# indygreg/python-zstandard

Hardware: NVIDIA H100
Metric: uncompressed GB/s (compress+decompress) (higher is better)
Workload: dtype u8

## Files before the change

### python_zstandard_b200/csrc/zb_common.cuh

```cuda
#pragma once
#include <cstdint>
#include <cstring>
#include <cuda_runtime.h>

typedef uint8_t  u8;
typedef uint16_t u16;
typedef uint32_t u32;
typedef uint64_t u64;

enum : u32 {
    ZB_OK = 0,
    ZB_E_GENERIC = 1,
    ZB_E_PREFIX_UNKNOWN = 10,
    ZB_E_FRAMEPARAM_UNSUPPORTED = 14,
    ZB_E_WINDOW_TOO_LARGE = 16,
    ZB_E_CORRUPTION = 20,
    ZB_E_CHECKSUM_WRONG = 22,
    ZB_E_LITERALS_HEADER_WRONG = 24,
    ZB_E_DICT_CORRUPTED = 30,
    ZB_E_DICT_WRONG = 32,
    ZB_E_TABLELOG_TOO_LARGE = 44,
    ZB_E_MAXSYMBOL_TOO_SMALL = 48,
    ZB_E_MEMORY = 64,
    ZB_E_DSTSIZE_TOO_SMALL = 70,
    ZB_E_SRCSIZE_WRONG = 72,
    ZB_E_UNKNOWN_SIZE = 200,
    ZB_E_SIZE_MISMATCH = 201,
};

#define ZB_MAGIC       0xFD2FB528u
#define ZB_MAGIC_DICT  0xEC30A437u
#define ZB_MAGIC_SKIP  0x184D2A50u
#define ZB_BLOCK_MAX   (128u << 10)
#define ZB_CONTENT_UNKNOWN 0xFFFFFFFFFFFFFFFFull

struct ZbSegment { u64 offset, length; };

#ifdef ZB_SIMT_EMULATION
#define ZB_LAUNCH(kernel, grid, block, smem, stream, ...) simt::launch((grid), (block), [&] { kernel(__VA_ARGS__); })
#else
#define ZB_LAUNCH(kernel, grid, block, smem, stream, ...) do { \
        if (smem) cudaFuncSetAttribute(kernel, cudaFuncAttributeMaxDynamicSharedMemorySize, (int)(smem)); \
        kernel<<<(grid), (block), (smem), (stream)>>>(__VA_ARGS__); } while (0)
#endif

static inline u32 zb_block_max(u32 window_log) { return window_log && window_log < 17 ? (1u << window_log) : ZB_BLOCK_MAX; }

template <class Seg, class JobVec, class InfoVec>
static inline u32 zb_cut_blocks(const Seg* segs, size_t n, u32 block_max, JobVec& jobs, InfoVec& info)
{
    u32 max_block = 0;
    for (size_t i = 0; i < n; i++) {
        u64 const len = segs[i].length; u64 pos = 0;
        info[i].first_job = jobs.size(); info[i].n_jobs = 0; info[i].pad = 0;
        while (pos < len) {
            u32 const sz = (u32)(len - pos < block_max ? len - pos : block_max);
            typename JobVec::value_type j;
            j.src_pos = segs[i].offset + pos; j.size = sz; j.seg = (u32)i; j.first = pos == 0; j.last = pos + sz == len;
            jobs.push_back(j); info[i].n_jobs++; pos += sz;
            if (sz > max_block) max_block = sz;
        }
    }
    return max_block;
}

static inline u64 zb_slot_bytes(u32 max_block) { return ((u64)max_block + (max_block >> 7) + 64 + 15) & ~15ull; }

struct ZbDictView { const u8* tail; u32 D; };
static inline ZbDictView zb_dict_view(const u8* content, u32 content_size)
{
    u32 const D = content_size < 32768u ? content_size : 32768u;
    ZbDictView v; v.tail = content + (content_size - D); v.D = D >= 8 ? D : 0;
    return v;
}

#define ZE_CHAIN_STEP 4u
static inline u64 zb_chain_positions(u64 len) { return len >= 8 ? (len - 8) / ZE_CHAIN_STEP + 1 : 0; }
static inline u32 zb_chain_log(u64 len)
{
    u64 const npos = zb_chain_positions(len);
    u32 L = 4; while ((1ull << L) < 4 * npos) L++;
    return L;
}
template <class Seg, class Desc, class JobVec, class InfoVec>
static inline void zb_chain_plan(const Seg* chunks, size_t m, Desc* cs, u64* tab_off, u64* pos_off, JobVec& jobs, InfoVec& info)
{
// ... 27 lines not shown
    return k > n_frames ? n_frames : k;
}
static inline u32 zb_chunk_cut(u32 n_frames, u32 k, u32 n_chunks) { return (u32)((u64)n_frames * k / n_chunks); }

struct ZbChunkShape { u32 warps, take, ctas; };
static inline ZbChunkShape zb_chunk_shape(u64 out_bytes, u32 n_frames, u32 sm_count)
{
    u64 const avg_out = out_bytes / (n_frames ? n_frames : 1);
    ZbChunkShape s;
    s.warps = avg_out <= (8u << 10) ? 8u : 7u;
    s.take = avg_out <= (8u << 10) ? 32u : (avg_out <= (16u << 10) ? 16u : (avg_out <= (32u << 10) ? 8u : (avg_out <= (64u << 10) ? 4u : 3u)));
    { u32 const spread = (n_frames + sm_count * s.warps - 1) / (sm_count * s.warps); if (s.take > spread) s.take = spread ? spread : 1; }
    s.ctas = sm_count; { u32 const need = (n_frames + s.warps * s.take - 1) / (s.warps * s.take); if (s.ctas > need) s.ctas = need; if (s.ctas == 0) s.ctas = 1; }
    return s;
}

struct ZbFrameInfo {
    u64 content_size;
    u64 n_seq_rec;
    u64 n_lit;
    u32 n_blocks;
    u32 status;
    u32 dict_id;
    u32 flags;
};

#define ZB_FAR_WINDOW  ((1ull << 31) - (1ull << 27))
#define ZB_FAR_DICT    (1ull << 27)

struct ZbFramePlace {
    u64 dst_off;
    u64 dst_cap;
    u64 blk_off;
    u64 seq_off;
    u64 lit_off;
};

enum : u32 { ZB_BLK_RAW = 0, ZB_BLK_RLE = 1, ZB_BLK_COMPRESSED = 2 };
enum : u32 { ZB_LIT_RAW = 0, ZB_LIT_RLE = 1, ZB_LIT_SCRATCH = 2 };

struct ZbBlock {
    u64 out_pos;
    u64 src_pos;
    u64 seq_pos;
    u32 kind;
    u32 regen;
    u32 lit_kind;
    u32 n_lit;
    u32 n_seq;
    u32 lit_byte;
};

typedef uint4 ZbSeq;

typedef u32 ZbFseCell;
#define ZB_CELL(next, nb, add, sym) ((u32)(next) | ((u32)(nb) << 10) | ((u32)(add) << 14) | ((u32)(sym) << 19))
#define ZB_CELL_NEXT(c) ((c) & 1023u)
#define ZB_CELL_NB(c)   (((c) >> 10) & 15u)
#define ZB_CELL_ADD(c)  (((c) >> 14) & 31u)
#define ZB_CELL_SYM(c)  ((c) >> 19)
#define ZB_CELL16(sym, x) ((u16)((sym) | ((x) << 6)))

struct ZbDictDev {
    const u8* content; u32 content_size; u32 dict_id;
    const u16* huf; u32 huf_log; u32 has_entropy;
    const ZbFseCell* ll; const ZbFseCell* of; const ZbFseCell* ml;
    u32 ll_log, of_log, ml_log;
    u32 rep[3];
};

struct ZbDictDigest {
    u16 huf[4096]; ZbFseCell ll[512]; ZbFseCell ml[512]; ZbFseCell of[256];
    u32 huf_log, ll_log, of_log, ml_log; u32 rep[3]; u32 dict_id; u32 content_off; u32 status; u32 has_entropy; u32 pad;
    short c_norm_ll[36], c_norm_of[32], c_norm_ml[54]; u32 c_max_ll, c_max_of, c_max_ml;
    u8 c_huf_nb[256]; u32 c_huf_max;
};

__device__ __forceinline__ u32 zb_rd16(const u8* p) { return (u32)p[0] | ((u32)p[1] << 8); }
__device__ __forceinline__ u32 zb_rd24(const u8* p) { return zb_rd16(p) | ((u32)p[2] << 16); }
__device__ __forceinline__ u32 zb_rd32(const u8* p) { return zb_rd16(p) | (zb_rd16(p + 2) << 16); }
__device__ __forceinline__ u64 zb_rd64(const u8* p) { return (u64)zb_rd32(p) | ((u64)zb_rd32(p + 4) << 32); }
__device__ __forceinline__ int zb_hibit(u32 v) { return 31 - __clz(v); }

__device__ __forceinline__ void zb_cp16(u8* sdst, const u8* gsrc)
{
#ifdef __CUDA_ARCH__
    asm volatile("cp.async.cg.shared.global [%0], [%1], 16;" :: "r"((u32)__cvta_generic_to_shared(sdst)), "l"(gsrc) : "memory");
#else
    memcpy(sdst, gsrc, 16);
#endif
}
__device__ __forceinline__ void zb_cp_commit()
{
#ifdef __CUDA_ARCH__
    asm volatile("cp.async.commit_group;" ::: "memory");
#endif
}
template <int N> __device__ __forceinline__ void zb_cp_wait()
{
#ifdef __CUDA_ARCH__
    asm volatile("cp.async.wait_group %0;" :: "n"(N) : "memory");
#endif
}

#ifdef __CUDA_ARCH__
#define ZB_RING_ARG(name) u8* name
#else
#define ZB_RING_ARG(name) u8* name = nullptr
#endif
template <int D>
struct ZbBitR {
    static_assert(D >= 2 && (D & (D - 1)) == 0, "ring depth: a power of two");
    const u8* c; u8* ring; int widx; u32 hi, lo; int avail; u32 nx0, nx1; int skew_bits; int lo_c; u32 n_;
#ifndef __CUDA_ARCH__
    alignas(16) u8 own[16 * D];
#endif

    __device__ __forceinline__ u32 word(int j) const { return *(const u32*)(ring + ((u32)j & (4u * D - 1)) * 4u); }
    __device__ __forceinline__ void fetch(int k) { zb_cp16(ring + ((u32)k & (D - 1)) * 16u, c + 16 * k); }
    __device__ __forceinline__ ~ZbBitR() { zb_cp_wait<0>(); }

    __device__ __forceinline__ bool start(const u8* s, u32 n, u8* ring_) {
        if (n == 0) return false;
#ifdef __CUDA_ARCH__
        ring = ring_;
#else
        ring = ring_ ? ring_ : own;
#endif
        c = (const u8*)((uintptr_t)s & ~(uintptr_t)15);
        int const skew = (int)(s - c);
        skew_bits = skew * 8; n_ = n;
        int const top = (skew + (int)n - 1) >> 4;
        #pragma unroll
        for (int q = 0; q < D; q++) if (top - q >= 0) fetch(top - q);
        zb_cp_commit();
        lo_c = top - D + 1 > 0 ? top - D + 1 : 0;
        return true;
    }
    __device__ __forceinline__ bool finish() {
        zb_cp_wait<0>();
        int const e = skew_bits / 8 + (int)n_ - 1;
        u32 const last = ring[(u32)e & (16u * D - 1)];
        if (last == 0) return false;
        int const P = e * 8 + zb_hibit(last);
        nx0 = nx1 = 0; lo = 0;
        if (P == 0) { hi = 0; avail = 0; widx = -1; return true; }
        int const wi = (P - 1) >> 5, k = P - wi * 32;
        hi = word(wi) << (32 - k); avail = k; widx = wi - 1;
        if (widx >= 0) nx0 = word(widx);
        if (widx >= 1) nx1 = word(widx - 1);
        refill();
        return true;
    }
    __device__ __forceinline__ bool init(const u8* s, u32 n, u8* ring_) { return start(s, n, ring_) && finish(); }
    __device__ __forceinline__ void refill() {
        zb_cp_wait<4 * D - 8>();
        bool const r = (avail <= 32) & (widx >= 0);
        u32 const a = (u32)avail;
        u32 const add_hi = __funnelshift_rc(nx0, 0u, a);
        u32 const new_lo = __funnelshift_lc(0u, nx0, 32u - a);
        hi |= r ? add_hi : 0u;
        lo = r ? new_lo : lo;
        avail += r ? 32 : 0;
        widx -= r ? 1 : 0;
        nx0 = r ? nx1 : nx0;
        if (r && widx >= 1) nx1 = word(widx - 1);
        int const t = ((widx - 1) >> 2) + 1 - D;
        if (t >= 0 && t < lo_c) { fetch(t); lo_c = t; }
        zb_cp_commit();
    }
    __device__ __forceinline__ u32 peek(u32 nb) const { return __funnelshift_rc(hi, 0u, 32u - nb); }
    __device__ __forceinline__ void skip(u32 nb) {
        hi = __funnelshift_lc(lo, hi, nb); lo = __funnelshift_lc(0u, lo, nb); avail -= (int)nb;
    }
    __device__ __forceinline__ u32 read(u32 nb) { u32 const v = peek(nb); skip(nb); return v; }
    __device__ __forceinline__ int left() const { return avail + 32 * (widx + 1) - skew_bits; }
};
```

### python_zstandard_b200/csrc/zb_entropy.cuh

```cuda
#pragma once

#define ZB_ENT_WS_BYTES   256
#define ZB_ENT_WS_STRIDE  (ZB_ENT_WS_BYTES + 16)
#define ZB_ENT_SKEW(b)    ((((b) + 15u) & ~15u) | 16u)
#define ZB_ENT_DEF_LL     512
#define ZB_ENT_DEF_OF     (ZB_ENT_DEF_LL + 2 * 64)
#define ZB_ENT_DEF_ML     (ZB_ENT_DEF_OF + 2 * 32)
#define ZB_ENT_HEAD_BYTES (ZB_ENT_DEF_ML + 2 * 64)
#define ZB_ENT_POOL_BYTES(W) ((((227 * 1024 - ZB_ENT_HEAD_BYTES) / (W))) & ~15)
#define ZB_ENT_SMEM(W)    ((W) * ZB_ENT_POOL_BYTES(W) + ZB_ENT_HEAD_BYTES)

enum : u32 { ZB_SRC_NONE = 0, ZB_SRC_PREDEF = 1, ZB_SRC_RLE = 2, ZB_SRC_NCOUNT = 3, ZB_SRC_DICT = 4 };
struct ZbTabSrc { u32 kind; u32 sym; const u8* p; u32 n; };

enum : u32 { ZB_BD_FIRST = 1, ZB_BD_FSE_VALID = 2, ZB_BD_SKIP = 4 };
struct ZbBlkDesc {
    u64 hdr_off;
    u64 seq_off, lit_off;
    u32 span;
    u32 frame;
    u32 flags;
    u32 block_max;
    ZbTabSrc dHuf, dLL, dOF, dML;
};
// ... 94 lines not shown
#define ZB_HUF_COARSE 8u
struct ZbHufTab { const u16* cells; u32 log, shift, T, base; };
__device__ __forceinline__ void zb_huf_shape(u32 log, ZbRank const& rank, u32& shift, u32& T, u32& base, u32& bytes)
{
    shift = log > ZB_HUF_COARSE ? log - ZB_HUF_COARSE : 0u;
    T = 0;
    #pragma unroll
    for (u32 wt = 1; wt <= 12 - ZB_HUF_COARSE; wt++) T += wt <= shift ? rank[wt] << (wt - 1) : 0u;
    base = (T + 3u) & ~3u;
    bytes = 2u * (base + (1u << (log - shift)));
}
__device__ __forceinline__ ZbHufTab zb_huf_full(const u16* cells, u32 log) { ZbHufTab t; t.cells = cells; t.log = log; t.shift = 0; t.T = 0; t.base = 0; return t; }
#define ZB_HCELL(t, v) ((t).cells[(v) < (t).T ? (v) : (t).base + ((v) >> (t).shift)])

__device__ static void zb_huf_fill(u16* cells, const u8* ws, u32 log, u32 nsym, ZbRank const& rank, u32 shift, u32 base)
{
    ZbPacked<6, 16> next; next.clear();
    {
        u32 p = 0;
        #pragma unroll
        for (u32 wt = 1; wt <= 12; wt++) { next.add(wt - 1, p); p += wt <= log ? (rank[wt] << (wt - 1)) : 0; }
    }
    for (u32 i = 0; i < nsym; i++) {
        u32 const wt = (ws[i >> 1] >> ((i & 1) * 4)) & 15; if (!wt) continue;
        u32 len = 1u << (wt - 1), p = next.get(wt - 1); next.add(wt - 1, len);
        if (wt > shift) { len >>= shift; p = base + (p >> shift); }
        u32 const cell = i | ((log + 1 - wt) << 8);
        if (len >= 4) { u64 const v = cell * 0x0001000100010001ull; u64* q = (u64*)(cells + p); for (u32 k = 0; k < len / 4; k++) q[k] = v; }
        else if (len == 2) *(u32*)(cells + p) = cell * 0x00010001u;
        else cells[p] = (u16)cell;
    }
}

#ifdef ZB_SIMT_EMULATION
__device__ __forceinline__ ZbRank zb_rank_pack(const u32* rank) { ZbRank r; r.clear(); for (u32 wt = 1; wt <= 12; wt++) r.add(wt - 1, rank[wt]); return r; }
__device__ static u32 zb_huf_weights(u8* ws, const u8* s, u32 n, u32& out_log, u32& out_nsym, u32* rank, ZB_RING_ARG(ring))
{
    ZbRank r; u32 const used = zb_huf_weights(ws, s, n, out_log, out_nsym, r, ring);
    rank[0] = used ? out_nsym : 0;
    for (u32 w = 1; w <= 12; w++) { rank[w] = used ? r[w] : 0; rank[0] -= rank[w]; }
    return used;
}
__device__ __forceinline__ void zb_huf_shape(u32 log, const u32* rank, u32& shift, u32& T, u32& base, u32& bytes)
{
    zb_huf_shape(log, zb_rank_pack(rank), shift, T, base, bytes);
}
__device__ static void zb_huf_fill(u16* cells, const u8* ws, u32 log, u32 nsym, const u32* rank, u32 shift, u32 base)
{
    zb_huf_fill(cells, ws, log, nsym, zb_rank_pack(rank), shift, base);
}
#endif

__device__ static bool zb_huf_stream2(u8* out, u32 n_out, const u8* s, u32 n, ZbHufTab const t, u8* ring)
{
    ZbBitR<4> b;
    if (!b.init(s, n, ring)) return false;
    u32 const log = t.log;
    u32 i = 0;
    while (i < n_out && ((uintptr_t)(out + i) & 3)) { u32 v = b.peek(log); u32 c = ZB_HCELL(t, v); out[i++] = (u8)c; b.skip(c >> 8); b.refill(); }
    for (; i + 4 <= n_out; i += 4) {
        u32 v0 = b.peek(log); u32 c0 = ZB_HCELL(t, v0); b.skip(c0 >> 8);
        u32 v1 = b.peek(log); u32 c1 = ZB_HCELL(t, v1); b.skip(c1 >> 8); b.refill();
        u32 v2 = b.peek(log); u32 c2 = ZB_HCELL(t, v2); b.skip(c2 >> 8);
        u32 v3 = b.peek(log); u32 c3 = ZB_HCELL(t, v3); b.skip(c3 >> 8); b.refill();
        *(u32*)(out + i) = (c0 & 255) | ((c1 & 255) << 8) | ((c2 & 255) << 16) | (c3 << 24);
    }
    for (; i < n_out; i++) { u32 v = b.peek(log); u32 c = ZB_HCELL(t, v); out[i] = (u8)c; b.skip(c >> 8); b.refill(); }
    return b.left() == 0;
}

struct ZbHufLane { ZbBitR<4> b; u8* out; u32 left; };

__device__ __forceinline__ void zb_huf_one(ZbHufLane& h, ZbHufTab const& t)
{
    u32 const v = h.b.peek(t.log); u32 const c = ZB_HCELL(t, v); *h.out++ = (u8)c; h.b.skip(c >> 8); h.b.refill(); h.left--;
}
#define ZB_HUF4(h) do { \
        u32 const v0_ = h.b.peek(t.log); u32 const c0_ = ZB_HCELL(t, v0_); h.b.skip(c0_ >> 8); \
        u32 const v1_ = h.b.peek(t.log); u32 const c1_ = ZB_HCELL(t, v1_); h.b.skip(c1_ >> 8); h.b.refill(); \
        u32 const v2_ = h.b.peek(t.log); u32 const c2_ = ZB_HCELL(t, v2_); h.b.skip(c2_ >> 8); \
        u32 const v3_ = h.b.peek(t.log); u32 const c3_ = ZB_HCELL(t, v3_); h.b.skip(c3_ >> 8); h.b.refill(); \
        *(u32*)h.out = (c0_ & 255) | ((c1_ & 255) << 8) | ((c2_ & 255) << 16) | (c3_ << 24); h.out += 4; h.left -= 4; } while (0)

__device__ static bool zb_huf_block(u8* dstl, u32 regen, const u8* p, u32 left, bool single, ZbHufTab const t, ZB_RING_ARG(ring))
{
    if (single) return zb_huf_stream2(dstl, regen, p, left, t, ring);
    if (left < 10) return false;
    u32 const l1 = zb_rd16(p), l2 = zb_rd16(p + 2), l3 = zb_rd16(p + 4), seg = (regen + 3) / 4;
    if (6 + l1 + l2 + l3 > left || seg * 3 > regen) return false;
    u32 const l4 = left - 6 - l1 - l2 - l3;
    ZbHufLane h0, h1, h2, h3;
    u8* const r1 = ring ? ring + 64 : nullptr; u8* const r2 = ring ? ring + 128 : nullptr; u8* const r3 = ring ? ring + 192 : nullptr;
    if (!h0.b.start(p + 6, l1, ring) || !h1.b.start(p + 6 + l1, l2, r1) || !h2.b.start(p + 6 + l1 + l2, l3, r2) || !h3.b.start(p + 6 + l1 + l2 + l3, l4, r3)) return false;
    if (!h0.b.finish() || !h1.b.finish() || !h2.b.finish() || !h3.b.finish()) return false;
    h0.out = dstl; h1.out = dstl + seg; h2.out = dstl + 2 * seg; h3.out = dstl + 3 * seg;
    h0.left = h1.left = h2.left = seg; h3.left = regen - 3 * seg;
    while (h0.left && ((uintptr_t)h0.out & 3)) zb_huf_one(h0, t);
    while (h1.left && ((uintptr_t)h1.out & 3)) zb_huf_one(h1, t);
    while (h2.left && ((uintptr_t)h2.out & 3)) zb_huf_one(h2, t);
    while (h3.left && ((uintptr_t)h3.out & 3)) zb_huf_one(h3, t);
    while (h0.left >= 4 && h1.left >= 4 && h2.left >= 4 && h3.left >= 4) { ZB_HUF4(h0); ZB_HUF4(h1); ZB_HUF4(h2); ZB_HUF4(h3); }
    while (h0.left >= 4) ZB_HUF4(h0);
    while (h1.left >= 4) ZB_HUF4(h1);
    while (h2.left >= 4) ZB_HUF4(h2);
    while (h3.left >= 4) ZB_HUF4(h3);
    while (h0.left) zb_huf_one(h0, t);
    while (h1.left) zb_huf_one(h1, t);
    while (h2.left) zb_huf_one(h2, t);
    while (h3.left) zb_huf_one(h3, t);
    return h0.b.left() == 0 && h1.b.left() == 0 && h2.b.left() == 0 && h3.b.left() == 0;
}

__device__ static int zb_seq_desc(ZbTabSrc& d, u32 mode, u32 max_sym_kind, u32 max_log, const u8* ip, u32 avail,
                                  bool repeat_ok, short* norm, u32& log, u32& max_sym, u32& need)
{
    int used = 0;
    if (mode == 0) { d.kind = ZB_SRC_PREDEF; }
    else if (mode == 1) { if (avail == 0 || ip[0] > max_sym_kind) return -1; d.kind = ZB_SRC_RLE; d.sym = ip[0]; used = 1; }
    else if (mode == 2) { d.kind = ZB_SRC_NCOUNT; d.p = ip; d.n = avail; }
    else if (!repeat_ok || d.kind == ZB_SRC_NONE) return -1;
    need = 0; log = 0; max_sym = max_sym_kind;
    if (d.kind == ZB_SRC_NCOUNT) {
        u32 const u = zb_read_ncount(norm, max_sym, log, d.p, d.n);
        if (u == 0 || log > max_log) return -1;
        if (mode == 2) { used = (int)u; d.n = u; }
        need = 2u << log;
    } else if (d.kind == ZB_SRC_RLE) need = 2;
    return used;
}

template <class F> __device__ __forceinline__ void zb_cta_for(u32 n, F f)
{
#ifdef __CUDA_ARCH__
    for (u32 i = threadIdx.x; i < n; i += blockDim.x) f(i);
#else
    if (threadIdx.x == 0) for (u32 i = 0; i < n; i++) f(i);
#endif
}

__device__ __forceinline__ void zb_cta_cells16(u8* dst, const ZbFseCell* src, u32 log)
{
    zb_cta_for(1u << log, [&](u32 i) { u32 const c = src[i]; ((u16*)dst)[i] = ZB_CELL16(ZB_CELL_SYM(c), (ZB_CELL_NEXT(c) + (1u << log)) >> ZB_CELL_NB(c)); });
}

template <int W>
__device__ __forceinline__ u32 zb_ent_head(u8* smem, ZbDictDev const& dict)
{
    u32* const lutLL = (u32*)smem; u32* const lutML = lutLL + 36;
    zb_cta_for(36, [&](u32 i) { lutLL[i] = c_LL_base[i] | ((u32)c_LL_bits[i] << 24); });
    zb_cta_for(53, [&](u32 i) { lutML[i] = c_ML_base[i] | ((u32)c_ML_bits[i] << 24); });
    zb_cta_cells16(smem + ZB_ENT_DEF_LL, g_defLL, 6);
    zb_cta_cells16(smem + ZB_ENT_DEF_OF, g_defOF, 5);
    zb_cta_cells16(smem + ZB_ENT_DEF_ML, g_defML, 6);
    u32 head = ZB_ENT_HEAD_BYTES;
    if (dict.has_entropy) {
        zb_cta_cells16(smem + head, dict.ll, dict.ll_log); head += 2u << dict.ll_log;
        zb_cta_cells16(smem + head, dict.of, dict.of_log); head += 2u << dict.of_log;
        zb_cta_cells16(smem + head, dict.ml, dict.ml_log); head += 2u << dict.ml_log;
    }
    __syncthreads();
    return ((ZB_ENT_SMEM(W) - head) / W) & ~15u;
}

#ifdef ZB_PHASE_TIMERS
__device__ unsigned long long g_zb_ent_phase[8];
#define ZB_EMARK(k) do { if (lane == 0) { long long const t_ = clock64(); atomicAdd(&g_zb_ent_phase[k], (unsigned long long)(t_ - t_ph)); t_ph = t_; } } while (0)
#elif defined(ZB_DEBUG_BLOCKS)
#define ZB_EMARK(k) do { if (err && !(t_ph & 1)) { printf("[emark %d] lane %u err %u\n", k, lane, err); t_ph |= 1; } } while (0)
#else
#define ZB_EMARK(k) do { (void)t_ph; } while (0)
#endif

template <bool SYMREP>
__device__ __forceinline__ u32 zb_seq_block(const u8* smem, u8* q, u8* ws, ZbDictDev const& dict,
                                            ZbTabSrc const& dLL, ZbTabSrc const& dOF, ZbTabSrc const& dML,
                                            u32 msLL, u32 msOF, u32 msML, u32 logLL, u32 logOF, u32 logML,
                                            const u8* ip, const u8* bend, u32 nseq, ZbSeq* sq, u32 n_lit, u64 room, u64 hist,
                                            u32& rep0, u32& rep1, u32& rep2, u32& lit_used, u32& produced, long long& t_ph)
{
    const u32* const lutLL = (const u32*)smem; const u32* const lutML = lutLL + 36;
    short* const normLL = (short*)ws; short* const normOF = normLL + 36; short* const normML = normOF + 32;
    u32 const dct_ll = ZB_ENT_HEAD_BYTES, dct_of = dct_ll + (2u << dict.ll_log), dct_ml = dct_of + (2u << dict.of_log);
    ZbTab tLL, tOF, tML;
    auto setup = [&](const ZbTabSrc& d, short* norm, u32 ms, u32 lg, int kind, u32 dct, u32 dlog, u32 def, u32 deflog, ZbTab& t) {
// ... 92 lines not shown
        bool done = lane >= take || !(f < n_frames) || status[f] != ZB_OK;

        const u8* s = src; u64 n = 0; ZbHdr h; ZbFramePlace pl; u32 err = ZB_OK;
        u64 cap = 0, out_pos = 0, blk_i = 0, seq_i = 0, lit_i = 0, pos = 0; u32 block_max = 0;
        u32 rep0 = 1, rep1 = 4, rep2 = 8;
        ZbTabSrc dHuf = {ZB_SRC_NONE, 0, nullptr, 0}, dLL = dHuf, dOF = dHuf, dML = dHuf;
        bool fse_valid = false;
        if (!done) {
            s = src + segs[f].offset; n = segs[f].length;
            zb_skip_skippable(s, n);
            zb_parse_header(s, n, h);
            pl = place[f]; cap = pl.dst_cap; blk_i = pl.blk_off; seq_i = pl.seq_off; lit_i = pl.lit_off; pos = h.hdr_size;
            block_max = h.window < ZB_BLOCK_MAX ? (u32)h.window : ZB_BLOCK_MAX;
            if (dict.has_entropy) {
                dHuf.kind = dLL.kind = dOF.kind = dML.kind = ZB_SRC_DICT; fse_valid = true;
                rep0 = dict.rep[0]; rep1 = dict.rep[1]; rep2 = dict.rep[2];
            }
            if (h.dict_id && dict.dict_id && h.dict_id != dict.dict_id) { err = ZB_E_DICT_WRONG; done = true; }
        }
        u64 const hist_extra = dict.content_size;

        long long t_ph = clock64() & ~1ll;
        while (__any_sync(0xFFFFFFFFu, !done)) {
            ZB_EMARK(0);
            ZbBlock B; B.kind = 0; B.regen = 0; B.n_seq = 0; B.n_lit = 0; B.lit_kind = 0; B.lit_byte = 0; B.src_pos = 0; B.seq_pos = seq_i; B.out_pos = out_pos;
            bool comp = false, last = false;
            u32 bsize = 0; const u8* bs = nullptr; const u8* bend = nullptr; const u8* ip = nullptr;
            ZbLitHdr L; L.type = 0; L.regen = 0; L.hdr = 0; L.csize = 0; L.single = 0;
            if (!done) {
                do {
                    if (pos + 3 > n) { err = ZB_E_SRCSIZE_WRONG; break; }
                    u32 const bh = zb_rd24(s + pos); pos += 3;
                    last = bh & 1; u32 const type = (bh >> 1) & 3; bsize = bh >> 3; B.kind = type;
                    if (type == 3) { err = ZB_E_CORRUPTION; break; }
                    if (type == ZB_BLK_RLE) {
                        if (pos + 1 > n) { err = ZB_E_SRCSIZE_WRONG; break; }
                        if (bsize > block_max) { err = ZB_E_CORRUPTION; break; }
                        if (bsize > cap - out_pos) { err = ZB_E_DSTSIZE_TOO_SMALL; break; }
                        B.src_pos = (u64)(s + pos - src); B.regen = bsize; B.lit_byte = s[pos]; pos += 1;
                    } else if (type == ZB_BLK_RAW) {
                        if (pos + bsize > n) { err = ZB_E_SRCSIZE_WRONG; break; }
                        if (bsize > block_max) { err = ZB_E_CORRUPTION; break; }
                        if (bsize > cap - out_pos) { err = ZB_E_DSTSIZE_TOO_SMALL; break; }
                        B.src_pos = (u64)(s + pos - src); B.regen = bsize; pos += bsize;
                    } else {
                        if (pos + bsize > n || bsize > block_max) { err = ZB_E_SRCSIZE_WRONG; break; }
                        bs = s + pos; bend = bs + bsize;
                        err = zb_parse_lit_header(bs, bsize, L);
                        if (err) break;
                        if (L.regen > block_max) { err = ZB_E_CORRUPTION; break; }
                        B.n_lit = L.regen; comp = true;
                    }
                } while (0);
                if (err) { done = true; comp = false; }
            }
            ZB_EMARK(1);
            bool wantH = false; u32 hlog = 0, hns = 0; ZbRank rank; const u8* hp = nullptr; u32 hleft = 0;
            if (comp) {
                do {
                    if (L.type == 0) {
                        if (L.hdr + L.regen > bsize) { err = ZB_E_CORRUPTION; break; }
                        B.lit_kind = ZB_LIT_RAW; B.src_pos = (u64)(bs + L.hdr - src); ip = bs + L.hdr + L.regen;
                    } else if (L.type == 1) {
                        if (L.hdr + 1 > bsize) { err = ZB_E_CORRUPTION; break; }
                        B.lit_kind = ZB_LIT_RLE; B.lit_byte = bs[L.hdr]; ip = bs + L.hdr + 1;
                    } else {
                        if (L.type == 3 && dHuf.kind == ZB_SRC_NONE) { err = ZB_E_DICT_CORRUPTED; break; }
                        if (!L.single && L.regen < 6) { err = ZB_E_LITERALS_HEADER_WRONG; break; }
                        if (L.csize + L.hdr > bsize || L.regen == 0) { err = ZB_E_CORRUPTION; break; }
                        hp = bs + L.hdr; hleft = L.csize;
                        if (L.type == 2) { dHuf.kind = ZB_SRC_NCOUNT; dHuf.p = hp; dHuf.n = hleft; }
                        if (dHuf.kind == ZB_SRC_NCOUNT) {
                            u32 const used = zb_huf_weights(ws, dHuf.p, dHuf.n, hlog, hns, rank, tabs + lane * 80);
                            if (used == 0 || (L.type == 2 && used >= hleft)) { err = ZB_E_CORRUPTION; break; }
                            if (L.type == 2) { hp += used; hleft -= used; dHuf.n = used; }
                            wantH = true;
                        }
                        B.lit_kind = ZB_LIT_SCRATCH; B.src_pos = lit_i; ip = bs + L.hdr + L.csize;
                    }
                } while (0);
                if (err) { done = true; comp = false; wantH = false; }
            }
            if (comp && B.lit_kind == ZB_LIT_SCRATCH && dHuf.kind == ZB_SRC_DICT) {
                if (!zb_huf_block(lits + lit_i, L.regen, hp, hleft, L.single, zb_huf_full(dict.huf, dict.huf_log), ws)) { err = ZB_E_CORRUPTION; done = true; comp = false; }
            }
            ZB_EMARK(2);
            {
                bool pending = wantH;
                u32 hshift = 0, hT = 0, hbase = 0, hbytes = 0;
                if (wantH) zb_huf_shape(hlog, rank, hshift, hT, hbase, hbytes);
                while (__any_sync(0xFFFFFFFFu, pending)) {
                    u32 const need = pending ? hbytes : 0;
                    u32 const incl = zb_warp_incl_scan((need + 15) & ~15u, lane);
                    if (pending && incl <= TAB_BYTES) {
                        u16* cells = (u16*)(tabs + incl - ((need + 15) & ~15u));
                        zb_huf_fill(cells, ws, hlog, hns, rank, hshift, hbase);
                        ZB_EMARK(6);
                        ZbHufTab t; t.cells = cells; t.log = hlog; t.shift = hshift; t.T = hT; t.base = hbase;
                        if (!zb_huf_block(lits + lit_i, L.regen, hp, hleft, L.single, t, ws)) { err = ZB_E_CORRUPTION; done = true; comp = false; }
                        pending = false;
                    }
                    __syncwarp();
                }
            }
            ZB_EMARK(3);
            if (comp && B.lit_kind == ZB_LIT_SCRATCH) lit_i += (L.regen + 15) & ~15u;
            u32 nseq = 0, logLL = 0, logOF = 0, logML = 0, msLL = 0, msOF = 0, msML = 0, needS = 0;
            short* const normLL = (short*)ws; short* const normOF = normLL + 36; short* const normML = normOF + 32;
            if (comp) {
                do {
                    if (ip >= bend) { err = ZB_E_SRCSIZE_WRONG; break; }
                    nseq = *ip++;
                    if (nseq > 0x7F) {
                        if (nseq == 0xFF) { if (ip + 2 > bend) { err = ZB_E_SRCSIZE_WRONG; break; } nseq = zb_rd16(ip) + 0x7F00; ip += 2; }
                        else { if (ip >= bend) { err = ZB_E_SRCSIZE_WRONG; break; } nseq = ((nseq - 0x80) << 8) + *ip++; }
                    }
                    B.n_seq = nseq;
                    if (nseq == 0) { if (ip != bend) err = ZB_E_CORRUPTION; break; }
                    if (ip + 1 > bend) { err = ZB_E_SRCSIZE_WRONG; break; }
                    u32 const modes = *ip++;
                    if (modes & 3) { err = ZB_E_CORRUPTION; break; }
                    u32 nd; int r;
                    r = zb_seq_desc(dLL, modes >> 6, 35, 9, ip, (u32)(bend - ip), fse_valid, normLL, logLL, msLL, nd);
                    if (r < 0) { err = ZB_E_CORRUPTION; break; } ip += r; needS += nd;
                    r = zb_seq_desc(dOF, (modes >> 4) & 3, 31, 8, ip, (u32)(bend - ip), fse_valid, normOF, logOF, msOF, nd);
                    if (r < 0) { err = ZB_E_CORRUPTION; break; } ip += r; needS += nd;
                    r = zb_seq_desc(dML, (modes >> 2) & 3, 52, 9, ip, (u32)(bend - ip), fse_valid, normML, logML, msML, nd);
                    if (r < 0) { err = ZB_E_CORRUPTION; break; } ip += r; needS += nd;
                    fse_valid = true;
                } while (0);
                if (err) { done = true; comp = false; nseq = 0; }
            }
            ZB_EMARK(4);
            u32 lit_used = 0, produced = 0;
            {
                bool pending = comp && nseq > 0;
                while (__any_sync(0xFFFFFFFFu, pending)) {
                    u32 const need = pending ? ZB_ENT_SKEW(needS) : 0;
                    u32 const incl = zb_warp_incl_scan(need, lane);
                    if (pending && incl <= TAB_BYTES) {
                        err = zb_seq_block<false>(zb_smem, tabs + incl - need, ws, dict, dLL, dOF, dML, msLL, msOF, msML, logLL, logOF, logML,
                                                   ip, bend, nseq, seqs + seq_i, L.regen, cap - out_pos, out_pos + hist_extra,
                                                   rep0, rep1, rep2, lit_used, produced, t_ph);
                        if (err) { done = true; comp = false; }
                        pending = false;
                    }
                    __syncwarp();
                }
            }
            ZB_EMARK(5);
            if (!done) {
                if (comp) {
                    seqs[seq_i + nseq] = make_uint4(lit_used, produced, 0, 0);
                    seq_i += nseq + 1;
                    u32 const tail = L.regen - lit_used;
                    if ((u64)produced + tail > cap - out_pos) err = ZB_E_DSTSIZE_TOO_SMALL;
                    B.regen = produced + tail;
                    if (!err && B.regen > block_max) err = ZB_E_CORRUPTION;
                    pos += bsize;
                }
                if (!err) {
                    blocks[blk_i++] = B;
                    out_pos += B.regen;
                    if (last) {
                        if (h.content_size != ZB_CONTENT_UNKNOWN && out_pos != h.content_size) err = ZB_E_CORRUPTION;
                        else if (h.checksum && pos + 4 > n) err = ZB_E_CHECKSUM_WRONG;
                        else {
                            if (h.checksum) ck_expect[f] = zb_rd32(s + pos);
                            if (dst_sizes && out_pos != cap) err = ZB_E_SIZE_MISMATCH;
                        }
                        done = true;
                    }
                }
                if (err) done = true;
            }
        }
        if (lane < take && f < n_frames && status[f] == ZB_OK) {
            if (err) { status[f] = err; out_sizes[f] = err == ZB_E_SIZE_MISMATCH ? out_pos : 0; } else out_sizes[f] = out_pos;
        } else if (lane < take && f < n_frames) out_sizes[f] = 0;
    }
}

// ... 16 lines not shown
        if (lane == 0) base = atomicAdd(work_counter, take);
        base = __shfl_sync(0xFFFFFFFFu, base, 0);
        if (base >= n_blocks) return;
        u32 const bi = base + lane;
        ZbBlkDesc D; D.frame = 0; D.flags = 0;
        if (lane < take && bi < n_blocks) D = bdesc[bi];
        bool done = lane >= take || !(bi < n_blocks) || (D.flags & ZB_BD_SKIP) || status[D.frame] != ZB_OK;

        const u8* s = src; u64 n = 0; u32 err = ZB_OK;
        u64 const cap = ~0ull >> 1; u64 out_pos = 0, blk_i = bi, seq_i = 0, lit_i = 0, pos = 0; u32 block_max = 0;
        u32 rep0 = 1, rep1 = 4, rep2 = 8;
        ZbTabSrc dHuf = {ZB_SRC_NONE, 0, nullptr, 0}, dLL = dHuf, dOF = dHuf, dML = dHuf;
        bool fse_valid = false;
        if (!done) {
            s = src + D.hdr_off; n = D.span; seq_i = D.seq_off; lit_i = D.lit_off; block_max = D.block_max;
            dHuf = D.dHuf; dLL = D.dLL; dOF = D.dOF; dML = D.dML; fse_valid = (D.flags & ZB_BD_FSE_VALID) != 0;
            if (D.flags & ZB_BD_FIRST) { if (dict.has_entropy) { rep0 = dict.rep[0]; rep1 = dict.rep[1]; rep2 = dict.rep[2]; } }
            else { rep0 = 0x80000000u; rep1 = 0xA0000000u; rep2 = 0xC0000000u; }
        }
        u64 const hist_extra = 1ull << 40;

        long long t_ph = clock64() & ~1ll;
        while (__any_sync(0xFFFFFFFFu, !done)) {
            ZB_EMARK(0);
            ZbBlock B; B.kind = 0; B.regen = 0; B.n_seq = 0; B.n_lit = 0; B.lit_kind = 0; B.lit_byte = 0; B.src_pos = 0; B.seq_pos = seq_i; B.out_pos = out_pos;
            bool comp = false, last = false;
            u32 bsize = 0; const u8* bs = nullptr; const u8* bend = nullptr; const u8* ip = nullptr;
            ZbLitHdr L; L.type = 0; L.regen = 0; L.hdr = 0; L.csize = 0; L.single = 0;
            if (!done) {
                do {
                    if (pos + 3 > n) { err = ZB_E_SRCSIZE_WRONG; break; }
                    u32 const bh = zb_rd24(s + pos); pos += 3;
                    last = bh & 1; u32 const type = (bh >> 1) & 3; bsize = bh >> 3; B.kind = type;
                    if (type == 3) { err = ZB_E_CORRUPTION; break; }
                    if (type == ZB_BLK_RLE) {
                        if (pos + 1 > n) { err = ZB_E_SRCSIZE_WRONG; break; }
                        if (bsize > block_max) { err = ZB_E_CORRUPTION; break; }
                        if (bsize > cap - out_pos) { err = ZB_E_DSTSIZE_TOO_SMALL; break; }
                        B.src_pos = (u64)(s + pos - src); B.regen = bsize; B.lit_byte = s[pos]; pos += 1;
                    } else if (type == ZB_BLK_RAW) {
                        if (pos + bsize > n) { err = ZB_E_SRCSIZE_WRONG; break; }
                        if (bsize > block_max) { err = ZB_E_CORRUPTION; break; }
                        if (bsize > cap - out_pos) { err = ZB_E_DSTSIZE_TOO_SMALL; break; }
                        B.src_pos = (u64)(s + pos - src); B.regen = bsize; pos += bsize;
                    } else {
                        if (pos + bsize > n || bsize > block_max) { err = ZB_E_SRCSIZE_WRONG; break; }
                        bs = s + pos; bend = bs + bsize;
                        err = zb_parse_lit_header(bs, bsize, L);
                        if (err) break;
                        if (L.regen > block_max) { err = ZB_E_CORRUPTION; break; }
                        B.n_lit = L.regen; comp = true;
                    }
                } while (0);
                if (err) { done = true; comp = false; }
            }
            ZB_EMARK(1);
            bool wantH = false; u32 hlog = 0, hns = 0; ZbRank rank; const u8* hp = nullptr; u32 hleft = 0;
            if (comp) {
                do {
                    if (L.type == 0) {
                        if (L.hdr + L.regen > bsize) { err = ZB_E_CORRUPTION; break; }
                        B.lit_kind = ZB_LIT_RAW; B.src_pos = (u64)(bs + L.hdr - src); ip = bs + L.hdr + L.regen;
                    } else if (L.type == 1) {
                        if (L.hdr + 1 > bsize) { err = ZB_E_CORRUPTION; break; }
                        B.lit_kind = ZB_LIT_RLE; B.lit_byte = bs[L.hdr]; ip = bs + L.hdr + 1;
                    } else {
                        if (L.type == 3 && dHuf.kind == ZB_SRC_NONE) { err = ZB_E_DICT_CORRUPTED; break; }
                        if (!L.single && L.regen < 6) { err = ZB_E_LITERALS_HEADER_WRONG; break; }
                        if (L.csize + L.hdr > bsize || L.regen == 0) { err = ZB_E_CORRUPTION; break; }
                        hp = bs + L.hdr; hleft = L.csize;
                        if (L.type == 2) { dHuf.kind = ZB_SRC_NCOUNT; dHuf.p = hp; dHuf.n = hleft; }
                        if (dHuf.kind == ZB_SRC_NCOUNT) {
                            u32 const used = zb_huf_weights(ws, dHuf.p, dHuf.n, hlog, hns, rank, tabs + lane * 64);
                            if (used == 0 || (L.type == 2 && used >= hleft)) { err = ZB_E_CORRUPTION; break; }
                            if (L.type == 2) { hp += used; hleft -= used; dHuf.n = used; }
                            wantH = true;
                        }
                        B.lit_kind = ZB_LIT_SCRATCH; B.src_pos = lit_i; ip = bs + L.hdr + L.csize;
                    }
                } while (0);
                if (err) { done = true; comp = false; wantH = false; }
            }
            if (comp && B.lit_kind == ZB_LIT_SCRATCH && dHuf.kind == ZB_SRC_DICT) {
                if (!zb_huf_block(lits + lit_i, L.regen, hp, hleft, L.single, zb_huf_full(dict.huf, dict.huf_log), ws)) { err = ZB_E_CORRUPTION; done = true; comp = false; }
            }
            ZB_EMARK(2);
            {
                bool pending = wantH;
                u32 hshift = 0, hT = 0, hbase = 0, hbytes = 0;
                if (wantH) zb_huf_shape(hlog, rank, hshift, hT, hbase, hbytes);
                while (__any_sync(0xFFFFFFFFu, pending)) {
                    u32 const need = pending ? hbytes : 0;
                    u32 const incl = zb_warp_incl_scan((need + 15) & ~15u, lane);
                    if (pending && incl <= TAB_BYTES) {
                        u16* cells = (u16*)(tabs + incl - ((need + 15) & ~15u));
                        zb_huf_fill(cells, ws, hlog, hns, rank, hshift, hbase);
                        ZB_EMARK(6);
                        ZbHufTab t; t.cells = cells; t.log = hlog; t.shift = hshift; t.T = hT; t.base = hbase;
                        if (!zb_huf_block(lits + lit_i, L.regen, hp, hleft, L.single, t, ws)) { err = ZB_E_CORRUPTION; done = true; comp = false; }
                        pending = false;
                    }
                    __syncwarp();
                }
            }
            ZB_EMARK(3);
            if (comp && B.lit_kind == ZB_LIT_SCRATCH) lit_i += (L.regen + 15) & ~15u;
            u32 nseq = 0, logLL = 0, logOF = 0, logML = 0, msLL = 0, msOF = 0, msML = 0, needS = 0;
            short* const normLL = (short*)ws; short* const normOF = normLL + 36; short* const normML = normOF + 32;
            if (comp) {
                do {
                    if (ip >= bend) { err = ZB_E_SRCSIZE_WRONG; break; }
                    nseq = *ip++;
                    if (nseq > 0x7F) {
                        if (nseq == 0xFF) { if (ip + 2 > bend) { err = ZB_E_SRCSIZE_WRONG; break; } nseq = zb_rd16(ip) + 0x7F00; ip += 2; }
                        else { if (ip >= bend) { err = ZB_E_SRCSIZE_WRONG; break; } nseq = ((nseq - 0x80) << 8) + *ip++; }
                    }
                    B.n_seq = nseq;
                    if (nseq == 0) { if (ip != bend) err = ZB_E_CORRUPTION; break; }
                    if (ip + 1 > bend) { err = ZB_E_SRCSIZE_WRONG; break; }
                    u32 const modes = *ip++;
                    if (modes & 3) { err = ZB_E_CORRUPTION; break; }
                    u32 nd; int r;
                    r = zb_seq_desc(dLL, modes >> 6, 35, 9, ip, (u32)(bend - ip), fse_valid, normLL, logLL, msLL, nd);
                    if (r < 0) { err = ZB_E_CORRUPTION; break; } ip += r; needS += nd;
                    r = zb_seq_desc(dOF, (modes >> 4) & 3, 31, 8, ip, (u32)(bend - ip), fse_valid, normOF, logOF, msOF, nd);
                    if (r < 0) { err = ZB_E_CORRUPTION; break; } ip += r; needS += nd;
                    r = zb_seq_desc(dML, (modes >> 2) & 3, 52, 9, ip, (u32)(bend - ip), fse_valid, normML, logML, msML, nd);
                    if (r < 0) { err = ZB_E_CORRUPTION; break; } ip += r; needS += nd;
                    fse_valid = true;
                } while (0);
                if (err) { done = true; comp = false; nseq = 0; }
            }
            ZB_EMARK(4);
            u32 lit_used = 0, produced = 0;
            {
                bool pending = comp && nseq > 0;
                while (__any_sync(0xFFFFFFFFu, pending)) {
                    u32 const need = pending ? ((needS + 15) & ~15u) : 0;
                    u32 const incl = zb_warp_incl_scan(need, lane);
                    if (pending && incl <= TAB_BYTES) {
                        err = zb_seq_block<true>(zb_smem, tabs + incl - need, ws, dict, dLL, dOF, dML, msLL, msOF, msML, logLL, logOF, logML,
                                                   ip, bend, nseq, seqs + seq_i, L.regen, cap - out_pos, out_pos + hist_extra,
                                                   rep0, rep1, rep2, lit_used, produced, t_ph);
                        if (err) { done = true; comp = false; }
                        pending = false;
                    }
                    __syncwarp();
                }
            }
            ZB_EMARK(5);
            if (!done) {
                if (comp) {
                    seqs[seq_i + nseq] = make_uint4(lit_used, produced, 0, 0);
                    seq_i += nseq + 1;
                    u32 const tail = L.regen - lit_used;
                    if ((u64)produced + tail > cap - out_pos) err = ZB_E_DSTSIZE_TOO_SMALL;
                    B.regen = produced + tail;
                    if (!err && B.regen > block_max) err = ZB_E_CORRUPTION;
                    pos += bsize;
                }
                if (!err) blocks[blk_i] = B;
                done = true;
            }
        }
        if (lane < take && bi < n_blocks && !(D.flags & ZB_BD_SKIP)) {
            ZbBlkExit X; X.rep[0] = rep0; X.rep[1] = rep1; X.rep[2] = rep2; X.err = err;
            bexit[bi] = X;
#ifdef ZB_DEBUG_BLOCKS
            if (err) printf("[entropy_blocks] block %u frame %u err %u flags %u span %u | huf k%u n%u | LL k%u n%u s%u | OF k%u n%u s%u | ML k%u n%u s%u | hdr %02x %02x %02x | LLp-src %lld\n", bi, D.frame, err, D.flags, D.span,
                            D.dHuf.kind, D.dHuf.n, D.dLL.kind, D.dLL.n, D.dLL.sym, D.dOF.kind, D.dOF.n, D.dOF.sym, D.dML.kind, D.dML.n, D.dML.sym,
                            src[D.hdr_off], src[D.hdr_off + 1], src[D.hdr_off + 2], D.dLL.p ? (long long)(D.dLL.p - src) : -1ll);
#endif
            if (err) atomicCAS(&status[D.frame], (u32)ZB_OK, err);
        }
    }
}
```

Measured before the change: 148.1.

## Batch Huffman 4-stream decode rounds by max table log with shared refills

Restructures the 4-stream Huffman literal decode loop so that each round decodes several symbols per stream (4, 3 or 2 depending on the largest table log across the warp) before refilling. All four bit readers then refill together under a single cp.async wait/commit pair instead of one per refill. The goal is to cut the wait/commit count and refill overhead and expose more independent table lookups across streams. A warp-wide max reduction picks a uniform round size so lanes do not diverge. It also adds a SIMT-emulation model of cp.async for host testing.

New measurement: 150.6, median of 6. +1.7%, better.

```diff
diff --git a/python_zstandard_b200/csrc/zb_common.cuh b/python_zstandard_b200/csrc/zb_common.cuh
--- a/python_zstandard_b200/csrc/zb_common.cuh
+++ b/python_zstandard_b200/csrc/zb_common.cuh
@@ -2,6 +2,10 @@
 #include <cstdint>
 #include <cstring>
 #include <cuda_runtime.h>
+#ifdef ZB_SIMT_EMULATION
+#include <deque>
+#include <vector>
+#endif
 
 typedef uint8_t  u8;
 typedef uint16_t u16;
@@ -195,10 +199,30 @@
 __device__ __forceinline__ u64 zb_rd64(const u8* p) { return (u64)zb_rd32(p) | ((u64)zb_rd32(p + 4) << 32); }
 __device__ __forceinline__ int zb_hibit(u32 v) { return 31 - __clz(v); }
 
+#ifdef ZB_SIMT_EMULATION
+struct ZbSimCopy { u8* dst; const u8* src; unsigned long long group; };
+struct ZbSimCopies { std::deque<ZbSimCopy> q; unsigned long long open = 0; };
+static inline ZbSimCopies& zb_sim_copies()
+{
+    static std::vector<ZbSimCopies> per_thread;
+    if (per_thread.size() <= threadIdx.x) per_thread.resize(threadIdx.x + 1);
+    return per_thread[threadIdx.x];
+}
+#define ZB_SIM_POISON 0xA5
+static inline unsigned __reduce_max_sync(unsigned mask, unsigned v)
+{
+    for (int d = 1; d < 32; d <<= 1) { unsigned const o = __shfl_xor_sync(mask, v, d); v = o > v ? o : v; }
+    return v;
+}
+#endif
 __device__ __forceinline__ void zb_cp16(u8* sdst, const u8* gsrc)
 {
 #ifdef __CUDA_ARCH__
     asm volatile("cp.async.cg.shared.global [%0], [%1], 16;" :: "r"((u32)__cvta_generic_to_shared(sdst)), "l"(gsrc) : "memory");
+#elif defined(ZB_SIMT_EMULATION)
+    ZbSimCopies& c = zb_sim_copies();
+    memset(sdst, ZB_SIM_POISON, 16);
+    c.q.push_back({sdst, gsrc, c.open});
 #else
     memcpy(sdst, gsrc, 16);
 #endif
@@ -207,12 +231,17 @@
 {
 #ifdef __CUDA_ARCH__
     asm volatile("cp.async.commit_group;" ::: "memory");
+#elif defined(ZB_SIMT_EMULATION)
+    zb_sim_copies().open++;
 #endif
 }
 template <int N> __device__ __forceinline__ void zb_cp_wait()
 {
 #ifdef __CUDA_ARCH__
     asm volatile("cp.async.wait_group %0;" :: "n"(N) : "memory");
+#elif defined(ZB_SIMT_EMULATION)
+    ZbSimCopies& c = zb_sim_copies();
+    while (!c.q.empty() && c.q.front().group + N < c.open) { memcpy(c.q.front().dst, c.q.front().src, 16); c.q.pop_front(); }
 #endif
 }
 
@@ -268,6 +297,10 @@
     __device__ __forceinline__ bool init(const u8* s, u32 n, u8* ring_) { return start(s, n, ring_) && finish(); }
     __device__ __forceinline__ void refill() {
         zb_cp_wait<4 * D - 8>();
+        refill_nc();
+        zb_cp_commit();
+    }
+    __device__ __forceinline__ void refill_nc() {
         bool const r = (avail <= 32) & (widx >= 0);
         u32 const a = (u32)avail;
         u32 const add_hi = __funnelshift_rc(nx0, 0u, a);
@@ -280,7 +313,6 @@
         if (r && widx >= 1) nx1 = word(widx - 1);
         int const t = ((widx - 1) >> 2) + 1 - D;
         if (t >= 0 && t < lo_c) { fetch(t); lo_c = t; }
-        zb_cp_commit();
     }
     __device__ __forceinline__ u32 peek(u32 nb) const { return __funnelshift_rc(hi, 0u, 32u - nb); }
     __device__ __forceinline__ void skip(u32 nb) {
diff --git a/python_zstandard_b200/csrc/zb_entropy.cuh b/python_zstandard_b200/csrc/zb_entropy.cuh
--- a/python_zstandard_b200/csrc/zb_entropy.cuh
+++ b/python_zstandard_b200/csrc/zb_entropy.cuh
@@ -200,7 +200,41 @@
         u32 const v3_ = h.b.peek(t.log); u32 const c3_ = ZB_HCELL(t, v3_); h.b.skip(c3_ >> 8); h.b.refill(); \
         *(u32*)h.out = (c0_ & 255) | ((c1_ & 255) << 8) | ((c2_ & 255) << 16) | (c3_ << 24); h.out += 4; h.left -= 4; } while (0)
 
-__device__ static bool zb_huf_block(u8* dstl, u32 regen, const u8* p, u32 left, bool single, ZbHufTab const t, ZB_RING_ARG(ring))
+__device__ __forceinline__ u32 zb_huf_sym(ZbBitR<4>& b, ZbHufTab const& t)
+{
+    u32 const v = b.peek(t.log); u32 const c = ZB_HCELL(t, v); b.skip(c >> 8); return c & 255u;
+}
+
+template <u32 K>
+__device__ __forceinline__ void zb_huf_rounds(ZbHufLane& h0, ZbHufLane& h1, ZbHufLane& h2, ZbHufLane& h3, ZbHufTab const& t)
+{
+    constexpr u32 S = K == 3 ? 12 : 4, W = S / 4;
+    while (h0.left >= S && h1.left >= S && h2.left >= S && h3.left >= S) {
+        u32 w0[W], w1[W], w2[W], w3[W];
+        #pragma unroll
+        for (u32 j = 0; j < W; j++) w0[j] = w1[j] = w2[j] = w3[j] = 0;
+        #pragma unroll
+        for (u32 r = 0; r < S / K; r++) {
+            #pragma unroll
+            for (u32 k = 0; k < K; k++) {
+                u32 const i = r * K + k, sh = 8 * (i & 3);
+                w0[i / 4] |= zb_huf_sym(h0.b, t) << sh;
+                w1[i / 4] |= zb_huf_sym(h1.b, t) << sh;
+                w2[i / 4] |= zb_huf_sym(h2.b, t) << sh;
+                w3[i / 4] |= zb_huf_sym(h3.b, t) << sh;
+            }
+            zb_cp_wait<4 * 4 - 8>();
+            h0.b.refill_nc(); h1.b.refill_nc(); h2.b.refill_nc(); h3.b.refill_nc();
+            zb_cp_commit();
+        }
+        #pragma unroll
+        for (u32 j = 0; j < W; j++) { ((u32*)h0.out)[j] = w0[j]; ((u32*)h1.out)[j] = w1[j]; ((u32*)h2.out)[j] = w2[j]; ((u32*)h3.out)[j] = w3[j]; }
+        h0.out += S; h1.out += S; h2.out += S; h3.out += S;
+        h0.left -= S; h1.left -= S; h2.left -= S; h3.left -= S;
+    }
+}
+
+__device__ static bool zb_huf_block(u8* dstl, u32 regen, const u8* p, u32 left, bool single, ZbHufTab const t, ZB_RING_ARG(ring), u32 maxlog = 0)
 {
     if (single) return zb_huf_stream2(dstl, regen, p, left, t, ring);
     if (left < 10) return false;
@@ -217,7 +251,10 @@
     while (h1.left && ((uintptr_t)h1.out & 3)) zb_huf_one(h1, t);
     while (h2.left && ((uintptr_t)h2.out & 3)) zb_huf_one(h2, t);
     while (h3.left && ((uintptr_t)h3.out & 3)) zb_huf_one(h3, t);
-    while (h0.left >= 4 && h1.left >= 4 && h2.left >= 4 && h3.left >= 4) { ZB_HUF4(h0); ZB_HUF4(h1); ZB_HUF4(h2); ZB_HUF4(h3); }
+    maxlog = maxlog > t.log ? maxlog : t.log;
+    if (maxlog <= 8) zb_huf_rounds<4>(h0, h1, h2, h3, t);
+    else if (maxlog <= 10) zb_huf_rounds<3>(h0, h1, h2, h3, t);
+    else zb_huf_rounds<2>(h0, h1, h2, h3, t);
     while (h0.left >= 4) ZB_HUF4(h0);
     while (h1.left >= 4) ZB_HUF4(h1);
     while (h2.left >= 4) ZB_HUF4(h2);
@@ -476,7 +513,7 @@
                 if (err) { done = true; comp = false; wantH = false; }
             }
             if (comp && B.lit_kind == ZB_LIT_SCRATCH && dHuf.kind == ZB_SRC_DICT) {
-                if (!zb_huf_block(lits + lit_i, L.regen, hp, hleft, L.single, zb_huf_full(dict.huf, dict.huf_log), ws)) { err = ZB_E_CORRUPTION; done = true; comp = false; }
+                if (!zb_huf_block(lits + lit_i, L.regen, hp, hleft, L.single, zb_huf_full(dict.huf, dict.huf_log), ws, dict.huf_log)) { err = ZB_E_CORRUPTION; done = true; comp = false; }
             }
             ZB_EMARK(2);
             {
@@ -486,12 +523,14 @@
                 while (__any_sync(0xFFFFFFFFu, pending)) {
                     u32 const need = pending ? hbytes : 0;
                     u32 const incl = zb_warp_incl_scan((need + 15) & ~15u, lane);
-                    if (pending && incl <= TAB_BYTES) {
+                    bool const go = pending && incl <= TAB_BYTES;
+                    u32 const maxlog = __reduce_max_sync(0xFFFFFFFFu, go ? hlog : 0u);
+                    if (go) {
                         u16* cells = (u16*)(tabs + incl - ((need + 15) & ~15u));
                         zb_huf_fill(cells, ws, hlog, hns, rank, hshift, hbase);
                         ZB_EMARK(6);
                         ZbHufTab t; t.cells = cells; t.log = hlog; t.shift = hshift; t.T = hT; t.base = hbase;
-                        if (!zb_huf_block(lits + lit_i, L.regen, hp, hleft, L.single, t, ws)) { err = ZB_E_CORRUPTION; done = true; comp = false; }
+                        if (!zb_huf_block(lits + lit_i, L.regen, hp, hleft, L.single, t, ws, maxlog)) { err = ZB_E_CORRUPTION; done = true; comp = false; }
                         pending = false;
                     }
                     __syncwarp();
@@ -674,7 +713,7 @@
                 if (err) { done = true; comp = false; wantH = false; }
             }
             if (comp && B.lit_kind == ZB_LIT_SCRATCH && dHuf.kind == ZB_SRC_DICT) {
-                if (!zb_huf_block(lits + lit_i, L.regen, hp, hleft, L.single, zb_huf_full(dict.huf, dict.huf_log), ws)) { err = ZB_E_CORRUPTION; done = true; comp = false; }
+                if (!zb_huf_block(lits + lit_i, L.regen, hp, hleft, L.single, zb_huf_full(dict.huf, dict.huf_log), ws, dict.huf_log)) { err = ZB_E_CORRUPTION; done = true; comp = false; }
             }
             ZB_EMARK(2);
             {
@@ -684,12 +723,14 @@
                 while (__any_sync(0xFFFFFFFFu, pending)) {
                     u32 const need = pending ? hbytes : 0;
                     u32 const incl = zb_warp_incl_scan((need + 15) & ~15u, lane);
-                    if (pending && incl <= TAB_BYTES) {
+                    bool const go = pending && incl <= TAB_BYTES;
+                    u32 const maxlog = __reduce_max_sync(0xFFFFFFFFu, go ? hlog : 0u);
+                    if (go) {
                         u16* cells = (u16*)(tabs + incl - ((need + 15) & ~15u));
                         zb_huf_fill(cells, ws, hlog, hns, rank, hshift, hbase);
                         ZB_EMARK(6);
                         ZbHufTab t; t.cells = cells; t.log = hlog; t.shift = hshift; t.T = hT; t.base = hbase;
-                        if (!zb_huf_block(lits + lit_i, L.regen, hp, hleft, L.single, t, ws)) { err = ZB_E_CORRUPTION; done = true; comp = false; }
+                        if (!zb_huf_block(lits + lit_i, L.regen, hp, hleft, L.single, t, ws, maxlog)) { err = ZB_E_CORRUPTION; done = true; comp = false; }
                         pending = false;
                     }
                     __syncwarp();
```
